# lzzcd001/MeshDiffusion

Measured on AMD Instinct MI355X. Metric: denoise steps/sec on 64^3x4 DMTet grids (sample-steps/s = n_gpus*batch*steps/wall), higher is better.
Workload: dtype f16f6 in the Winograd convs behind a GroupNorm (fp16 hi*hi MFMA + MX block-scaled e2m3 cross terms in a K-concatenated scaled MFMA at twice the e4m3 rate; operands and weights equalised per input channel by a power of two: md_wino_equaliser, after the load-time calibration from the measured operand

## Files before the change

include/meshdiffusion_hip.h:

```cpp
#ifndef MESHDIFFUSION_HIP_H
#define MESHDIFFUSION_HIP_H

#include <stdint.h>

#ifdef __cplusplus
extern "C" {
#endif

#define MD_OK 0
#define MD_ERR_BAD_ARG (-1)
#define MD_ERR_UNSUPPORTED (-2)
#define MD_ERR_NO_DEVICE (-3)

#define MD_ABI_VERSION 16

enum {
  MD_CFG_C3_128 = 0,
  MD_CFG_C3_128_K16 = 1,
  MD_CFG_C3_32 = 2,
  MD_CFG_C3_LOW = 3,
  MD_CFG_C3_S2 = 4,
  MD_CFG_G1_128 = 5,
  MD_CFG_G1_128_LOW = 6,
  MD_CFG_G1_64_LOW = 7,
// ... 129 lines not shown
int md_wino_prep_f6(const float* x1, const float* x2, int32_t c1, int32_t c2, const float* ac, int32_t silu, int32_t ups,
                    const float* eq, void* t_out, int32_t batch, int32_t D, int32_t H, int32_t W, void* stream);
int md_wino_pack_weights_f6(const float* w, const float* eq, void* wpk, int32_t cout, int32_t cin, int64_t s_row, int64_t s_k, void* stream);
int md_conv3_wino_f6(const void* t_in, const void* wpk, float* out, const float* bias, int64_t bias_bstride,
                     const float* residual, int64_t res_bstride, double* stats, int32_t batch, int32_t cin, int32_t cout,
                     int32_t D, int32_t H, int32_t W, void* stream);

int md_wino_prep_f6_nin(const float* x1, const float* x2, int32_t c1, int32_t c2, const float* ac, int32_t silu, const float* eq,
                        void* t_out, const void* wpk, const float* bias, float* res, int32_t batch, int32_t D, int32_t H, int32_t W,
                        int32_t n_cu, void* stream);

#define MD_WINO_FMT_BF16X3 0
#define MD_WINO_FMT_F16F8 1
#define MD_WINO_FMT_F16F6 2
int md_wino_prep_upsdh(int32_t fmt, const float* x1, const float* x2, int32_t c1, int32_t c2, const float* ac, int32_t silu,
                       const float* eq, void* t_out, int32_t batch, int32_t D, int32_t H, int32_t W, void* stream);
int md_conv3_wino_upsdh(int32_t fmt, const void* t_in, const void* wpk, float* out, const float* bias, int64_t bias_bstride,
                        const float* residual, int64_t res_bstride, double* stats, int32_t batch, int32_t cin, int32_t cout,
                        int32_t D, int32_t H, int32_t W, void* stream);

int md_conv3_wino_upsfold(int32_t fmt, const void* t_in, int32_t t_full, const void* wpk, float* out, const float* bias,
                          int64_t bias_bstride, const float* residual, int64_t res_bstride, double* stats, int32_t batch,
                          int32_t cin, int32_t cout, int32_t D, int32_t H, int32_t W, void* stream);

int md_conv3_stem(const void* x16, const void* wpk, float* out, const float* bias, const float* residual, double* stats,
                  int32_t batch, int32_t cout, int32_t D, int32_t H, int32_t W, void* stream);

int md_conv3_head(const float* x, const float* ac, const void* wpk, float* y, int32_t batch, int32_t cin, int32_t rows_alloc,
                  int32_t D, int32_t H, int32_t W, void* stream);

int md_conv3_stem_dgrad(const float* g0, const void* wpk, float* y, int32_t batch, int32_t cout, int32_t rows_alloc,
                        int32_t D, int32_t H, int32_t W, void* stream);

enum { MD_PACK_WPK = 0, MD_PACK_WINO = 1, MD_PACK_WINO_F6 = 2 };
typedef struct MdPackJob {
  const float* w;
  void* out;
  int64_t s_row, s_k, s_tap, n_items, block0;
  int32_t rows, kdim, taps, nt, kc, prec, flip, kind;
} MdPackJob;
int md_pack_batch(const MdPackJob* jobs_dev, int32_t n_jobs, int64_t total_blocks, int32_t tiled, void* stream);

int md_conv3_s2(const float* x, const void* wpk, float* out, const float* bias, int64_t bias_bstride, double* stats,
                int32_t batch, int32_t cin, int32_t rows, int32_t rows_alloc, int32_t D, int32_t H, int32_t W, void* stream);

int md_wino_prep_v2(const float* x1, const float* x2, int32_t c1, int32_t c2, const float* ac, int32_t silu, int32_t ups,
// ... 281 lines not shown
```

meshdiffusion_amd/csrc/conv3_wino.hip:

```cpp
#include <type_traits>
#include "md_common.h"
#include "md_pack.h"

namespace {
constexpr int WN_THREADS = 256;
constexpr int WN_TZ = 4, WN_TY = 8, WN_TX = 8;
constexpr int WN_TPOS = 6 * 10 * 4;
constexpr int WN_HBUF = 4 * WN_TPOS * 16;
constexpr int WN_NDMA = WN_HBUF / 1024;
constexpr int WN_RED = 4 * 32 * 2;
constexpr int WN_WAVE_LDS = 2 * WN_HBUF;
constexpr int WN_LDS_BYTES = 4 * WN_WAVE_LDS + 4 * WN_NDMA * 64 * 4;

__device__ const uint4 wn_zero16 = {0u, 0u, 0u, 0u};

typedef uint32_t wn_u32x4 __attribute__((ext_vector_type(4)));
__device__ __forceinline__ uint4 wn_gload16(const void* p) {
  return __builtin_bit_cast(uint4, *(__attribute__((address_space(1))) const wn_u32x4*)(uintptr_t)p);
}
}

__global__ __launch_bounds__(256) void md_wino_prep_kernel(const float* __restrict__ x1, const float* __restrict__ x2,
                                                           int c1, int c2, const float* __restrict__ ac, int silu, int ups,
                                                           uint4* __restrict__ T, int batch, int D, int H, int W,
// ... 114 lines not shown
  const float wscale = md_wino_f8_wscale(__uint_as_float(hdr[0]));
  if (id == 0) {
    hdr[1] = (uint32_t)ilogbf(wscale);
    hdr[2] = __float_as_uint(1.0f / wscale);
    hdr[3] = 6u;
  }
  if (id >= n) return;
  wpk[id] = md_pack_wino_f6_item(w, cout, cin, s_row, s_k, wscale, id, eq);
}

struct WnArgs {
  const uint4* T;
  const uint4* wpk;
  float* out;
  const float* bias;
  const float* residual;
  double* stats;
  const float* hdr;
  int64_t bias_bstride, res_bstride;
  int batch, cin, cout, D, H, W;
  float out_scale;
  const uint32_t* amax;
  int ups_dh;
};

typedef int wn_i32x8 __attribute__((ext_vector_type(8)));
typedef int wn_i32x4 __attribute__((ext_vector_type(4)));

template <int ABL, bool F8 = false, bool F6 = false, bool RES = false>
__global__ __launch_bounds__(WN_THREADS) void md_conv3_wino_kernel(const WnArgs A) {
  __shared__ __attribute__((aligned(16))) unsigned char wn_smem[WN_LDS_BYTES];
  const int tid = threadIdx.x, lane = tid & 63;
  const int wid = __builtin_amdgcn_readfirstlane(tid >> 6);
  const int j = lane & 31, h = lane >> 5;
  uint64_t stamp[12];
  auto mark = [&](int k) { if constexpr (ABL & 128) stamp[k] = __builtin_amdgcn_s_memtime(); };
  if constexpr (ABL & 128) stamp[10] = __builtin_amdgcn_s_memrealtime();
  mark(0);

#ifndef W8_STAGGER
#define W8_STAGGER 0
#endif
  if constexpr (W8_STAGGER > 0) {
    const unsigned lin = blockIdx.x + gridDim.x * blockIdx.y;
    if (lin < 256u) {
      const unsigned ph = (lin * 0x9E3779B1u) >> 24;
      const uint64_t t_end = __builtin_amdgcn_s_memtime() + ((uint64_t)ph * (uint64_t)W8_STAGGER >> 8);
      while (__builtin_amdgcn_s_memtime() < t_end) __builtin_amdgcn_s_sleep(16);
    }
  }
  const int D = A.D, H = A.H, W = A.W, Wp = W >> 1;
  const int64_t P = (int64_t)D * H * W, Ph = P >> (1 + 2 * A.ups_dh);
  const int ush = A.ups_dh, Hrows = H >> ush;
  const int ntx = W / WN_TX, nty = H / WN_TY, ntz = D / WN_TZ;
  const int tiles = ntx * nty * ntz;
  int bid = blockIdx.x;
  if ((gridDim.x & 7) == 0) bid = (blockIdx.x & 7) * (gridDim.x >> 3) + (blockIdx.x >> 3);
  const int b = bid / tiles, t = bid % tiles;
  const int x0 = (t % ntx) * WN_TX, y0 = ((t / ntx) % nty) * WN_TY, z0 = (t / (ntx * nty)) * WN_TZ;
  const int rtb = blockIdx.y;
  const int CG = A.cin >> 3, nchunk = A.cin >> 4;
  const int nsteps = nchunk * 9;

  unsigned char* my_smem = wn_smem + wid * WN_WAVE_LDS;

  auto halo_off = [&](int k) -> int {
    const int e = k * 64 + lane;
    const int hp = e / WN_TPOS, tp = e % WN_TPOS;
    const int dz = tp / 40, hy = (tp >> 2) % 10, pr = tp & 3;
    const int z = z0 + dz - 1, y = y0 + hy - 1;
    const bool live = (z >= 0) & (z < D) & (y >= 0) & (y < H);
    const int row = (z >> ush) * Hrows + (y >> ush);
    if constexpr (F8) {
      const int Phi = (int)Ph;
      const int off = (hp >> 1) * 8 * Phi + (hp & 1) * Phi + row * Wp + (x0 >> 1) + pr;
      return live ? off : -1;
    }
    return live ? (int)((int64_t)(hp >> 1) * 8 * Ph + (int64_t)(hp & 1) * Ph + (int64_t)row * Wp + (x0 >> 1) + pr) : -1;
  };
  const uint4* tbase = A.T + ((int64_t)b * CG * 8 + wid * 2) * Ph;
  const uint4* zsrc = &wn_zero16;
  auto halo_load = [&](int chunk, int k) -> uint4 {
    const int dk = halo_off(k);
    const uint4* src = dk >= 0 ? tbase + (int64_t)chunk * 16 * Ph + dk : zsrc;
    if constexpr (ABL & 32)
      src = A.T + (((blockIdx.x & 255) * 4 + wid) * 2 + (chunk & 1)) * 960 + k * 64 + lane;
    if constexpr (ABL & 64)
      src = A.T + ((((((int64_t)bid * 4 + wid) * nchunk + chunk) * 960) & (((int64_t)1 << 26) - 1)) + k * 64 + lane);
    if constexpr (ABL & 1) return make_uint4(0, 0, 0, 0);
    return wn_gload16(src);
  };
  auto halo_store = [&](int buf, int k, const uint4& v) {
    if constexpr (!(ABL & 1)) *(uint4*)(my_smem + buf * WN_HBUF + k * 1024 + lane * 16) = v;
  };
  const uint4* wbase = A.wpk + (((int64_t)rtb * nsteps) * 4 + wid) * 512 + lane;
  auto load_A = [&](int s, bf16x8 (&dst)[8]) {
    const uint4* wp = wbase + (int64_t)s * 2048;
#pragma unroll
    for (int i = 0; i < 8; ++i) dst[i] = __builtin_bit_cast(bf16x8, wp[i * 64]);
  };
  const unsigned char* vB = my_smem + h * 2 * WN_TPOS * 16 + j * 16;
  auto read_B = [&](int tap, int buf, bf16x8 (&dst)[8], bool force) {
    const int kd = tap / 3, kh = tap % 3;
    const unsigned char* p = vB + buf * WN_HBUF + (kd * 40 + kh * 4) * 16;
#pragma unroll
    for (int ct = 0; ct < 4; ++ct)
      if (force || !(ABL & 8)) {
        dst[ct * 2] = *(const bf16x8*)(p + ct * 40 * 16);
        dst[ct * 2 + 1] = *(const bf16x8*)(p + WN_TPOS * 16 + ct * 40 * 16);
      }
  };

  f32x16 acc[4][4];
  auto zero_acc = [&]() {
#pragma unroll
    for (int rt = 0; rt < 4; ++rt)
#pragma unroll
      for (int ct = 0; ct < 4; ++ct) {
#pragma unroll
        for (int r = 0; r < 16; ++r) acc[rt][ct][r] = 0.f;
        asm volatile("" : "+a"(acc[rt][ct]));
      }
  };
#ifndef W8_PRO_FENCE
#define W8_PRO_FENCE 1
#endif
  if constexpr (!W8_PRO_FENCE) zero_acc();
  float descale = 1.f;
  if constexpr (F8) {
    static_assert(ABL == 0 || ABL == 128, "timing ablations exist for the bf16x3 loop only");
#ifndef W8_HG
#define W8_HG 3
#endif
    auto slot3_of_store = [](int u) constexpr -> int { return (u == 0 || u == 3 || u == 6) ? 0 : ((u == 2 || u == 5 || u == 8) ? 1 : 2); };
    auto slot3_of_request = [](int u) constexpr -> int { return (u == 0 || u == 3 || u == 6) ? 0 : ((u == 2 || u == 5 || u == 8) ? 1 : 2); };
    const int npairs = nsteps >> 1;
    const uint4* wbase8 = A.wpk + (((int64_t)rtb * npairs) * 4 + wid) * 1024 + lane;
    uint4 A8h[2][4][2], B8h[2][2], hs8[W8_HG == 3 ? 3 : 2][4];
    wn_i32x8 A8f[2][4], B8f[2];
    uint32_t* otab = (uint32_t*)(wn_smem + 4 * WN_WAVE_LDS) + wid * (WN_NDMA * 64) + lane;
    static_assert(4 * WN_WAVE_LDS + 4 * WN_NDMA * 64 * 4 <= WN_LDS_BYTES, "offset tables fit behind the halo buffers");
    uint32_t live_mask = 0;
    constexpr int D1 = 64, D2 = (40 - 8) * 16, D3 = WN_HBUF - (2 * 40 + 2 * 4) * 16;
    const unsigned char* vBh = my_smem + h * 2 * WN_TPOS * 16 + j * 16;
    const unsigned char* vB8a = my_smem + WN_TPOS * 16 + j * 16 + h * D1;
    const unsigned char* vB8b = my_smem + WN_TPOS * 16 + j * 16 + h * D2;
    const unsigned char* vB8c = my_smem + WN_TPOS * 16 + j * 16 + h * D3;
    auto step_off = [](int s) constexpr -> int { return (s / 9) * WN_HBUF + (((s % 9) / 3) * 40 + ((s % 9) % 3) * 4) * 16; };
    auto cat8 = [](const uint4& x, const uint4& y) -> wn_i32x8 {
      const wn_i32x4 a = __builtin_bit_cast(wn_i32x4, x), b = __builtin_bit_cast(wn_i32x4, y);
      return __builtin_shufflevector(a, b, 0, 1, 2, 3, 4, 5, 6, 7);
    };
    auto halo_store8 = [&](int buf, int k, uint4 v) {
      const bool lv = (live_mask >> k) & 1u;
      v.x = lv ? v.x : 0u; v.y = lv ? v.y : 0u; v.z = lv ? v.z : 0u; v.w = lv ? v.w : 0u;
      *(uint4*)(my_smem + buf * WN_HBUF + k * 1024 + lane * 16) = v;
    };
    auto read_B8 = [&](auto uc, auto ctc, uint4 (&dh)[2], wn_i32x8& df) {
      constexpr int u = decltype(uc)::value, ct = decltype(ctc)::value;
      constexpr int o0 = step_off(2 * u) + ct * 40 * 16, o1 = step_off(2 * u + 1) + ct * 40 * 16, dk = o1 - o0;
// ... 254 lines not shown
        __builtin_amdgcn_sched_group_barrier(0x008, 2, 0);
        __builtin_amdgcn_sched_group_barrier(0x200, 1, 0);
        __builtin_amdgcn_sched_barrier(0);
      }
    }
  #undef WN_MFMA
  }

  mark(2);
  if constexpr (ABL & 16) {
    float keep = 0.f;
#pragma unroll
    for (int rt = 0; rt < 4; ++rt)
#pragma unroll
      for (int ct = 0; ct < 4; ++ct) keep += acc[rt][ct][0];
    if (keep == 123.456f) A.out[tid] = keep;
    return;
  }
  constexpr int XF_ITEMS = 1024, XREG_FLOATS = (4 * XF_ITEMS + 16) * 4;
  static_assert(2 * XREG_FLOATS * 4 + 2 * WN_RED * 4 <= WN_LDS_BYTES, "two exchange regions + the statistics area fit");
  float* xreg = (float*)wn_smem;
  float* red = xreg + 2 * XREG_FLOATS;
  const int rows_total = A.cout;
  float* outp = A.out + (int64_t)b * rows_total * P;
  const float* resp = A.residual ? A.residual + (int64_t)b * A.res_bstride : nullptr;
  const float* biasp = A.bias ? A.bias + (int64_t)b * A.bias_bstride : nullptr;
  const bool want_stats = (ABL & 128) ? false : A.stats != nullptr;
  const int half = lane & 1, xq = (lane >> 1) & 7, cgp = lane >> 4;
  const int cq = 2 * cgp + half, prr = xq >> 1;
  const bool odd = xq & 1;
  const float sgn = odd ? -1.f : 1.f;
  const int64_t gp0 = ((int64_t)(z0 + wid) * H + y0) * W + x0 + xq;
  auto flush_stats = [&](int r) {
    if (tid < 64) {
      const int ch = tid >> 1, which = tid & 1;
      const float* rb = red + (r & 1) * WN_RED;
      float sum = 0.f;
#pragma unroll
      for (int k = 0; k < 4; ++k) sum += rb[(k * 32 + ch) * 2 + which];
      const int row = rtb * 128 + r * 32 + ch;
      atomicAdd(A.stats + ((int64_t)b * rows_total + row) * 2 + which, (double)sum);
    }
  };
  const bool has_bias = biasp != nullptr;
  f32x4 pbias[4], pres[RES ? 2 : 1][8];
  auto prefetch_res = [&](int r) {
    if constexpr (RES) {
// ... 183 lines not shown
extern "C" int md_wino_pack_weights_f8(const float* w, const float* eq, void* wpk, int32_t cout, int32_t cin, int64_t s_row, int64_t s_k, void* stream) {
  return md_wino_pack_weights_f8_launch(false, w, eq, wpk, cout, cin, s_row, s_k, stream);
}

extern "C" int md_wino_pack_weights_f6(const float* w, const float* eq, void* wpk, int32_t cout, int32_t cin, int64_t s_row, int64_t s_k, void* stream) {
  return md_wino_pack_weights_f8_launch(true, w, eq, wpk, cout, cin, s_row, s_k, stream);
}

static int md_conv3_wino_f8_launch(bool f6, const void* t_in, const void* wpk, float* out, const float* bias, int64_t bias_bstride,
                                   const float* residual, int64_t res_bstride, double* stats, int32_t batch, int32_t cin,
                                   int32_t cout, int32_t D, int32_t H, int32_t W, void* stream, float out_scale = 1.0f,
                                   const uint32_t* amax = nullptr, bool upsdh = false) {
  if (!t_in || !wpk || !out || batch <= 0) return MD_ERR_BAD_ARG;
  if (cin <= 0 || cout <= 0 || (cin % 32) || (cout % 128)) return MD_ERR_UNSUPPORTED;
  if (D <= 0 || H <= 0 || W <= 0 || (D % WN_TZ) || (H % WN_TY) || (W % WN_TX)) return MD_ERR_UNSUPPORTED;
  if ((int64_t)D * H * W * 8 >= (int64_t)1 << 31) return MD_ERR_UNSUPPORTED;
  WnArgs a;
  a.T = (const uint4*)t_in; a.wpk = (const uint4*)wpk; a.out = out; a.bias = bias; a.residual = residual; a.stats = stats;
  a.hdr = (const float*)((const unsigned char*)wpk + (int64_t)cout * cin * 36 * 4);
  a.out_scale = out_scale; a.amax = amax;
  a.bias_bstride = bias_bstride; a.res_bstride = res_bstride;
  a.batch = batch; a.cin = cin; a.cout = cout; a.D = D; a.H = H; a.W = W;
  a.ups_dh = upsdh ? 1 : 0;
  const int tiles = (D / WN_TZ) * (H / WN_TY) * (W / WN_TX);
  const dim3 grid((unsigned)(tiles * batch), (unsigned)(cout / 128));
  MD_HIP_CLEAR_ERROR();
#ifdef W8_STAMPS
  constexpr int ABL_ = 128;
#else
  constexpr int ABL_ = 0;
#endif
#define WN_LAUNCH8(F6_, RES_) hipLaunchKernelGGL((md_conv3_wino_kernel<ABL_, true, F6_, RES_>), grid, dim3(WN_THREADS), 0, (hipStream_t)stream, a)
  if (f6) { if (residual) WN_LAUNCH8(true, true); else WN_LAUNCH8(true, false); }
  else { if (residual) WN_LAUNCH8(false, true); else WN_LAUNCH8(false, false); }
#undef WN_LAUNCH8
  MD_HIP_CHECK_LAUNCH();
  return MD_OK;
}

extern "C" int md_conv3_wino_f8(const void* t_in, const void* wpk, float* out, const float* bias, int64_t bias_bstride,
                                const float* residual, int64_t res_bstride, double* stats, int32_t batch, int32_t cin,
                                int32_t cout, int32_t D, int32_t H, int32_t W, void* stream) {
  return md_conv3_wino_f8_launch(false, t_in, wpk, out, bias, bias_bstride, residual, res_bstride, stats, batch, cin, cout, D, H, W, stream);
}

extern "C" int md_conv3_wino_f6(const void* t_in, const void* wpk, float* out, const float* bias, int64_t bias_bstride,
// ... 4 lines not shown

extern "C" int md_conv3_wino_f6_scaled(const void* t_in, const void* wpk, float* out, const float* bias, int64_t bias_bstride,
                                       const float* residual, int64_t res_bstride, double* stats, int32_t batch, int32_t cin,
                                       int32_t cout, int32_t D, int32_t H, int32_t W, float out_scale, const uint32_t* amax_bits, void* stream) {
  if (!(out_scale > 0.f)) return MD_ERR_BAD_ARG;
  return md_conv3_wino_f8_launch(true, t_in, wpk, out, bias, bias_bstride, residual, res_bstride, stats, batch, cin, cout, D, H, W, stream, out_scale,
                                 amax_bits);
}

static int md_conv3_wino_launch(const void* t_in, const void* wpk, float* out, const float* bias, int64_t bias_bstride,
                                const float* residual, int64_t res_bstride, double* stats, int32_t batch, int32_t cin,
                                int32_t cout, int32_t D, int32_t H, int32_t W, int32_t variant, void* stream, bool upsdh) {
  if (!t_in || !wpk || !out || batch <= 0) return MD_ERR_BAD_ARG;
  if (cin <= 0 || cout <= 0 || (cin % 32) || (cout % 128)) return MD_ERR_UNSUPPORTED;
  if (D <= 0 || H <= 0 || W <= 0 || (D % WN_TZ) || (H % WN_TY) || (W % WN_TX)) return MD_ERR_UNSUPPORTED;
  if ((int64_t)D * H * W * 8 >= (int64_t)1 << 31) return MD_ERR_UNSUPPORTED;
  WnArgs a;
  a.T = (const uint4*)t_in; a.wpk = (const uint4*)wpk; a.out = out; a.bias = bias; a.residual = residual; a.stats = stats;
  a.hdr = nullptr;
  a.out_scale = 1.0f; a.amax = nullptr;
  a.bias_bstride = bias_bstride; a.res_bstride = res_bstride;
  a.batch = batch; a.cin = cin; a.cout = cout; a.D = D; a.H = H; a.W = W;
  a.ups_dh = upsdh ? 1 : 0;
  const int tiles = (D / WN_TZ) * (H / WN_TY) * (W / WN_TX);
  MD_HIP_CLEAR_ERROR();
  const dim3 grid((unsigned)(tiles * batch), (unsigned)(cout / 128));
#define WN_LAUNCH(A_) hipLaunchKernelGGL((md_conv3_wino_kernel<A_, false, false, true>), grid, dim3(WN_THREADS), 0, (hipStream_t)stream, a)
  if (variant != 0 && residual == nullptr) return MD_ERR_UNSUPPORTED;
  if (upsdh && variant != 0) return MD_ERR_BAD_ARG;
  switch (variant) {
    case 0:
      if (residual) WN_LAUNCH(0);
      else hipLaunchKernelGGL((md_conv3_wino_kernel<0, false, false, false>), grid, dim3(WN_THREADS), 0, (hipStream_t)stream, a);
      break;
#ifdef MD_BUILD_ABLATIONS
    case 1: WN_LAUNCH(1); break;
    case 2: WN_LAUNCH(2); break;
    case 4: WN_LAUNCH(4); break;
    case 6: WN_LAUNCH(6); break;
    case 22: WN_LAUNCH(22); break;
    case 9: WN_LAUNCH(9); break;
    case 16: WN_LAUNCH(16); break;
    case 25: WN_LAUNCH(25); break;
    case 32: WN_LAUNCH(32); break;
    case 64: WN_LAUNCH(64); break;
    case 128: WN_LAUNCH(128); break;
#endif
    default: return MD_ERR_UNSUPPORTED;
  }
#undef WN_LAUNCH
  MD_HIP_CHECK_LAUNCH();
  return MD_OK;
}

extern "C" int md_conv3_wino(const void* t_in, const void* wpk, float* out, const float* bias, int64_t bias_bstride,
                             const float* residual, int64_t res_bstride, double* stats, int32_t batch, int32_t cin,
                             int32_t cout, int32_t D, int32_t H, int32_t W, int32_t variant, void* stream) {
  return md_conv3_wino_launch(t_in, wpk, out, bias, bias_bstride, residual, res_bstride, stats, batch, cin, cout, D, H, W, variant, stream, false);
}

extern "C" int md_conv3_wino_upsdh(int32_t fmt, const void* t_in, const void* wpk, float* out, const float* bias, int64_t bias_bstride,
                                   const float* residual, int64_t res_bstride, double* stats, int32_t batch, int32_t cin,
                                   int32_t cout, int32_t D, int32_t H, int32_t W, void* stream) {
  if (fmt == MD_WINO_FMT_BF16X3)
    return md_conv3_wino_launch(t_in, wpk, out, bias, bias_bstride, residual, res_bstride, stats, batch, cin, cout, D, H, W, 0, stream, true);
  if (fmt != MD_WINO_FMT_F16F8 && fmt != MD_WINO_FMT_F16F6) return MD_ERR_BAD_ARG;
  return md_conv3_wino_f8_launch(fmt == MD_WINO_FMT_F16F6, t_in, wpk, out, bias, bias_bstride, residual, res_bstride, stats, batch, cin, cout, D, H,
                                 W, stream, 1.0f, nullptr, true);
}
```

meshdiffusion_amd/csrc/gemm_conv.hip:

```cpp
#include "md_common.h"
#include "md_pack.h"

template <int NT_, int KC_, int TZ_, int TY_, int TX_, int TAPS_, int STRIDE_, int WR_, int WC_,
          int SW_ = 0, int PIPE_ = 0, int ABL_ = 0, int BF_ = 0>
struct GCfg {
  static constexpr int BF = BF_;
  static constexpr int ABL = ABL_;
  static constexpr int NT = NT_, KC = KC_, TZ = TZ_, TY = TY_, TX = TX_, TAPS = TAPS_,
                       STRIDE = STRIDE_, WR = WR_, WC = WC_, SW = SW_, PIPE = PIPE_;
  static constexpr int MT = TZ * TY * TX;
  static constexpr int NW = WR * WC;
  static constexpr int NTHREADS = NW * 64;
  static constexpr int RM = NT / (32 * WR);
  static constexpr int CM = MT / (32 * WC);
  static constexpr int KSZ = (TAPS == 125 || TAPS == 25) ? 5 : (TAPS == 27 || TAPS == 9) ? 3 : 1;
  static constexpr int KSX = (TAPS == 25 || TAPS == 9) ? 1 : KSZ;
  static constexpr int ZH = (TAPS > 1) ? (TZ - 1) * STRIDE + KSZ : 1;
  static constexpr int YH = (TAPS > 1) ? (TY - 1) * STRIDE + KSZ : 1;
  static constexpr int XH = (TAPS > 1) ? (TX - 1) * STRIDE + KSX : MT;
  static constexpr int XHP = XH;
  static constexpr int HS = (SW == 1) ? ((ZH + 1) / 2) * YH * 24 : ZH * YH * XHP;
  static constexpr int HPOS = ZH * YH * XH;
  static __device__ __forceinline__ int slot_of(int hz, int hy, int hx) {
    if constexpr (SW == 1) return (hz >> 1) * (YH * 24) + hy * 24 + (hz & 1) * 12 + hx;
// ... 541 lines not shown
  }
  __syncthreads();
  if (threadIdx.x < 16) {
    const float t = (red[0][threadIdx.x] + red[1][threadIdx.x]) + (red[2][threadIdx.x] + red[3][threadIdx.x]);
    A.stats[((int64_t)b * A.rows_alloc + cg * 8) * 2 + threadIdx.x] += (double)t;
  }
}

int md_launch_splitk_reduce(const MdGemmConvArgs& a, hipStream_t stream) {
  const int64_t P = (int64_t)a.D * a.H * a.W;
  if (a.stats != nullptr) {
    MD_HIP_CLEAR_ERROR();
    hipLaunchKernelGGL(md_splitk_reduce_stats_kernel, dim3((unsigned)(a.batch * (a.rows_alloc / 8))), dim3(256), 0, stream, a, P);
    MD_HIP_CHECK_LAUNCH();
    return MD_OK;
  }
  const int64_t n4 = (int64_t)a.batch * (a.rows_alloc / 8) * P * 2;
  int blocks = (int)((n4 + 255) / 256);
  if (blocks > 2048) blocks = 2048;
  MD_HIP_CLEAR_ERROR();
  hipLaunchKernelGGL(md_splitk_reduce_kernel, dim3((unsigned)blocks), dim3(256), 0, stream, a, P);
  MD_HIP_CHECK_LAUNCH();
  return MD_OK;
}

extern "C" int64_t md_gemm_conv_partial_bytes(const MdGemmConvArgs* a) {
  if (a == nullptr) return MD_ERR_BAD_ARG;
  if (a->ksplit <= 1) return 0;
  return (int64_t)a->ksplit * a->batch * (a->rows_alloc / 8) * ((int64_t)a->D * a->H * a->W) * 8 * 4;
}

template <class C>
static int launch_cfg(const MdGemmConvArgs& a, hipStream_t stream) {
  if (a.kdim % C::KC != 0 || a.kdim <= 0) return MD_ERR_BAD_ARG;
  if (a.rows <= 0 || a.rows_alloc % 8 != 0 || a.batch <= 0) return MD_ERR_BAD_ARG;
  int tiles;
  if (C::TAPS > 1) {
    if (a.D % C::TZ || a.H % C::TY || a.W % C::TX) return MD_ERR_BAD_ARG;
    if (a.ups && ((a.D | a.H | a.W) & 1)) return MD_ERR_BAD_ARG;
    if (a.ups && C::STRIDE != 1) return MD_ERR_BAD_ARG;
    tiles = (a.D / C::TZ) * (a.H / C::TY) * (a.W / C::TX);
  } else {
    if (a.D != 1 || a.H != 1 || a.W % C::MT || a.ups) return MD_ERR_BAD_ARG;
    tiles = a.W / C::MT;
  }
  if (a.a_src == MD_A_S16B && a.a_rows <= 0) return MD_ERR_BAD_ARG;
// ... 137 lines not shown
```

meshdiffusion_amd/hip_ops.py:

```python
import ctypes as C
import math
import os

import torch

from . import _lib
from ._lib import (A_PACKED, A_S16B, PREC_BF16X3, PREC_FP16X2, CFG_C3_128, CFG_C3_128_V2, CFG_C3_128_SW, CFG_C3_128_PIPE, CFG_C3_128_FAST, CFG_C5_128_K16, CFG_C5_32_K16, CFG_C3_128_W4, CFG_C3X_32, CFG_C5X_32_K16, CFG_C3X_128_K16, CFG_C5X_128, CFG_G1_128_N128, CFG_C3_128_K16, CFG_C3_32, CFG_C3_LOW, CFG_C3_S2,
                   CFG_G1_128, CFG_G1_128_LOW, CFG_G1_64_LOW, CFG_NT_KC, OUT_F32B, OUT_NCDHW, OUT_S16B,
                   MdGemmConvArgs, check)


CFG_ABL1, CFG_ABL2, CFG_ABL3, CFG_ABL4, CFG_ABL5 = 101, 102, 103, 104, 105
CFG_F1, CFG_F3, CFG_F4, CFG_F6, CFG_F7, CFG_F8 = 111, 113, 114, 116, 117, 118
CFG_FAST_EC = 122
_MODES = ("bf16x3", "fp16x2", "f16f8", "f16f6")
DEFAULT_PRECISION = os.environ.get("MD_PRECISION", "bf16x3")
FORCE_PRECISION = os.environ.get("MD_FORCE_PRECISION")
WINO_EQ = os.environ.get("MD_WINO_EQ", "1") == "1"


def _decode(mode):
    if mode not in _MODES:
        raise ValueError(f"unknown precision mode {mode!r}")
    return ("bf16x3", mode[3:]) if mode in ("f16f8", "f16f6") else (mode, False)
# ... 465 lines not shown
CALIBRATE = None


def wino_operand_ms(parts, ac, silu, B, P):
    lib = _lib.load()
    assert 1 <= len(parts) <= 2
    cin = sum(c for _, c in parts)
    x2, c2 = (parts[1][0], parts[1][1]) if len(parts) == 2 else (None, 0)
    ms = torch.zeros(cin, dtype=torch.float32, device=parts[0][0].device)
    check(lib.md_wino_operand_ms(_ptr(parts[0][0]), _ptr(x2), parts[0][1], c2, _ptr(ac), 1 if silu else 0, B, P, _ptr(ms), _stream()),
          "md_wino_operand_ms")
    return ms


WINO_MIN_WGS = 128
WINO_MIN_WGS_TRAIN = 256


def wino_ok(rows, kdim, S, B):
    return (WINO and PRECISION == "bf16x3" and rows % 128 == 0 and kdim % 32 == 0 and S % 8 == 0
            and B * (S ** 3 // 256) * (rows // 128) >= (max(WINO_MIN_WGS, WINO_MIN_WGS_TRAIN) if TRAINING_SCOPE else WINO_MIN_WGS))


def wgrad_nin_ok(co, ci, P):
    return co % 128 == 0 and ci % 128 == 0 and P % 16 == 0


def wgrad_nin(dy_s16, x_s16, B, co, ci, P, dw, ksplit=None):
    lib = _lib.load()
    units = (co // 128) * (ci // 128)
    if ksplit is None:
        ksplit = max(1, min(256 // units, B * P // 16 // 8))
    nbytes = lib.md_wgrad_nin_workspace_bytes(co, ci, ksplit)
    if nbytes <= 0:
        raise _lib.MeshDiffusionHipError("md_wgrad_nin_workspace_bytes: unsupported shape")
    ws = torch.empty(nbytes // 4, dtype=torch.float32, device=dy_s16.device)
    ev = _prof_begin()
    check(lib.md_wgrad_nin(_ptr(dy_s16), _ptr(x_s16), _ptr(dw), _ptr(ws), nbytes, B, co, ci, P, ksplit, 1, co, _stream()),
          "md_wgrad_nin")
    _prof_end(ev, "wgrad_nin", 2.0 * B * co * ci * P, 4.0 * B * (co + ci) * P, f"{ci}->{co}@{P}")


_WINO_SCRATCH = {}


def _wino_scratch(n_bf16, device, slot="t"):
# ... 146 lines not shown


def conv3_wino_upsfold(wf, t, B, S, *, bias=None, bias_bstride=0, stats=None, out=None, dims=None):
    lib = _lib.load()
    D, H, W = dims if dims is not None else (S, S, S)
    P = D * H * W
    assert isinstance(wf, WinoWeightF8) and wf.fmt == "f6" and wf.rows % 4 == 0
    rows = wf.rows // 4
    t_fmt = getattr(t, "_md_fmt", None)
    if t_fmt is not None:
        if t_fmt != "f6" or not getattr(t, "_md_ups", False) or getattr(t, "_md_eq", 0) != (wf.eq.data_ptr() if wf.eq is not None else 0):
            raise _lib.MeshDiffusionHipError(f"conv3_wino_upsfold: operand (format {t_fmt!r}) does not belong to these weights")
    if out is None:
        out = f32b_empty(B, rows, P, t.device)
    ev = _prof_begin()
    check(lib.md_conv3_wino_upsfold(_lib.WINO_FMT["f6"], _ptr(t), 0 if getattr(t, "_md_compact", False) else 1, _ptr(wf.data), _ptr(out),
                                    _ptr(bias), bias_bstride, None, 0, _ptr(stats), B, wf.kdim, rows, D, H, W, _stream()),
          "md_conv3_wino_upsfold")
    _prof_end(ev, "wino", 2.0 * B * rows * wf.kdim * 27 * P, 4.0 * (2 * B * wf.kdim * P // 4 + wf.rows * wf.kdim * 36 + B * rows * P),
              f"{wf.kdim}->{rows}@{D}x{H}x{W}" + ("/stats" if stats is not None else "") + "/fold/f6")
    return out


CFG_S2_PACK = CFG_C3_128_K16
S2_MIN_WGS = 100


def conv3_s2_ok(rows, kdim, S_out, B=None):
    ok = PRECISION == "bf16x3" and kdim % 32 == 0 and rows % 8 == 0 and S_out % 8 == 0
    return ok and (B is None or B * (S_out ** 3 // 256) * ((rows + 127) // 128) >= S2_MIN_WGS)


def conv3_s2(pw, x, B, S_out, *, bias=None, bias_bstride=0, stats=None, out=None, dims=None):
    lib = _lib.load()
    D, H, W = dims if dims is not None else (S_out, S_out, S_out)
    P = D * H * W
    rows_alloc = ((pw.rows + 7) // 8) * 8
    if out is None:
        out = f32b_empty(B, rows_alloc, P, x.device)
    ev = _prof_begin()
    check(lib.md_conv3_s2(_ptr(x), _ptr(pw.data), _ptr(out), _ptr(bias), bias_bstride, _ptr(stats), B, pw.kdim, pw.rows,
                          rows_alloc, D, H, W, _stream()), "md_conv3_s2")
    _prof_end(ev, "s2", 2.0 * B * pw.rows * pw.kdim * 27 * P, 4.0 * (B * pw.kdim * 8 * P + pw.rows * pw.kdim * 27 + B * pw.rows * P),
              f"{pw.kdim}->{pw.rows}@{D}x{H}x{W}" + ("/stats" if stats is not None else ""))
    return out

# ... 539 lines not shown
```

meshdiffusion_amd/lib/diffusion/models/layers.py:

```python
import math
from typing import NamedTuple

import numpy as np
import torch
import torch.nn as nn

from .... import hip_ops as ops


def variance_scaling(scale, mode, distribution, in_axis=1, out_axis=0, dtype=torch.float32, device="cpu"):
    def init(shape, dtype=dtype, device=device):
        receptive = np.prod(shape) / shape[in_axis] / shape[out_axis]
        fan_in, fan_out = shape[in_axis] * receptive, shape[out_axis] * receptive
        denom = {"fan_in": fan_in, "fan_out": fan_out, "fan_avg": (fan_in + fan_out) / 2}[mode]
        var = scale / denom
        if distribution == "normal":
            return torch.randn(*shape, dtype=dtype, device=device) * np.sqrt(var)
        if distribution == "uniform":
            return (torch.rand(*shape, dtype=dtype, device=device) * 2.0 - 1.0) * np.sqrt(3 * var)
        raise ValueError("invalid distribution for variance scaling initializer")

    return init


# ... 108 lines not shown


def fused_operand_ok(pw, ups=0):
    cfgs = (ops.CFG_C3_128_FAST,) if ups else (ops.CFG_C3_128_FAST, ops.CFG_C3_LOW)
    return ops.FUSE_GN_APPLY and pw.cfg in cfgs and pw.prec == ops.PREC_BF16X3


class Conv3Plan(NamedTuple):
    path: str
    fmt: object
    compact: bool
    shortcut_in_pass: bool
    keep: bool
    stats: bool
    ksplit: int
    fused_loader: bool
    ups_fold: bool = False


def plan_conv3(pw, operand, B, S_out, *, ups, out_mode, rows_alloc, want_stats, wino):
    P = S_out ** 3
    plain = out_mode == ops.OUT_F32B and rows_alloc == pw.rows
    sums = bool(want_stats and ops.FUSE_GN_STATS and plain)
    if (operand is not None and wino is not None and plain and pw.prec == ops.PREC_BF16X3
            and ops.wino_ok(pw.rows, pw.kdim, S_out, B)):
        infer = not (operand.wino_only or operand.drop or operand.keep)
        fmt = infer and ops.wino_f8_ok(
            S_out, parts=operand.parts, normalised=operand.ac is not None
            or (ops.WINO_EQ and hasattr(wino, "measured") and wino.measured() is not None))
        owner = getattr(wino, "owner", None)
        if fmt and owner is not None and wino.site in getattr(owner, "md_bf16x3_sites", ()):
            fmt = False
        compact = infer and ops.prep_compact_ok(ups, S_out, S_out, S_out)
        shortcut = bool(operand.nin is not None and fmt == "f6" and not compact and not ups
                        and ops.block_pass_ok(operand.parts, operand.nin[0].rows, B, S_out, S_out, S_out))
        fold = bool(infer and hasattr(wino, "fold") and ops.ups_fold_ok(ups, fmt, pw.rows, B, S_out, S_out, S_out))
        return Conv3Plan("wino", fmt, compact, shortcut, operand.keep, sums, 1, False, fold)
    ksplit = ops.ksplit_for(pw.cfg, B, pw.rows, pw.kdim, S_out) if out_mode == ops.OUT_F32B else 1
    sums = sums and ((pw.cfg == ops.CFG_C3_128_FAST and ksplit == 1) or (ksplit > 1 and P <= 512 and B * rows_alloc >= 2048))
    return Conv3Plan("direct", False, False, False, False, sums, ksplit, operand is not None and not operand.wino_only)


def run_conv3(pw, act_s16, B, S_out, *, bias=None, bias_bstride=0, residual=None, res_bstride=None, ups=0,
              out=None, out_mode=ops.OUT_F32B, rows_alloc=None, want_stats=False, b_f32=None, wino=None):
    P = S_out ** 3
    b_f32 = ops.F32Operand.of(b_f32)
    dev = act_s16.device if act_s16 is not None else b_f32.parts[0][0].device
    rows_alloc = rows_alloc if rows_alloc is not None else ((pw.rows + 7) // 8) * 8
    if out is None:
        out = ops.f32b_empty(B, rows_alloc, P, dev)
    if residual is not None and res_bstride is None:
        res_bstride = rows_alloc * P
    if b_f32 is not None:
        b_f32.t_kept = b_f32.shortcut = None
    plan = plan_conv3(pw, b_f32, B, S_out, ups=ups, out_mode=out_mode, rows_alloc=rows_alloc, want_stats=want_stats, wino=wino)
    stats = ops.stats_zeros(B, rows_alloc, dev) if plan.stats else None
    if plan.path == "wino":
        _conv3_wino(plan, pw, b_f32, wino, B, S_out, ups, out, stats, bias=bias, bias_bstride=bias_bstride, residual=residual,
                    res_bstride=res_bstride or 0)
    else:
# ... 6 lines not shown
    elif hasattr(out, "_md_sums"):
        del out._md_sums
    return out


def _conv3_wino(plan, pw, op, wino, B, S_out, ups, out, stats, **epilogue):
    owner = getattr(wino, "owner", None)
    if ops.CALIBRATE is not None and owner is not None and not op.wino_only:
        ms = ops.wino_operand_ms(op.parts, op.ac, op.silu, B, op.parts[0][0].shape[2])
        rec = ops.CALIBRATE.setdefault((id(owner), wino.site), [owner, wino.site, torch.zeros_like(ms), 0])
        rec[2] += ms
        rec[3] += 1
    eq = wino.eq() if plan.fmt and hasattr(wino, "eq") else None
    if plan.shortcut_in_pass:
        t, op.shortcut = ops.wino_prep_nin(op.parts, op.ac, op.silu, B, S_out, eq, op.nin[0], op.nin[1])
    else:
        t = ops.wino_prep(op.parts, op.ac, op.silu, ups, B, S_out, drop=op.drop, keep=plan.keep, f8=plan.fmt, eq=eq, compact=plan.compact)
    if plan.keep:
        op.t_kept = t
    if plan.ups_fold:
        assert epilogue.get("residual") is None, "md_conv3_wino_upsfold has no residual operand"
        ops.conv3_wino_upsfold(wino.fold(), t, B, S_out, stats=stats, out=out, bias=epilogue.get("bias"),
                               bias_bstride=epilogue.get("bias_bstride", 0))
    else:
        ops.conv3_wino(wino(plan.fmt) if plan.fmt else wino(), t, B, S_out, stats=stats, out=out, **epilogue)
    if plan.fmt and ops.AUDIT is not None:
        t3 = ops.wino_prep(op.parts, op.ac, op.silu, ups, B, S_out, compact=plan.compact)
        ref = ops.conv3_wino(wino(), t3, B, S_out, **epilogue)
        ops.AUDIT.append(dict(owner=owner, site=getattr(wino, "site", None), fmt=plan.fmt, cin=pw.kdim, cout=pw.rows,
                              S=S_out, rel_l2=float((torch.linalg.vector_norm(out - ref, dtype=torch.float64)
                                                     / torch.linalg.vector_norm(ref, dtype=torch.float64).clamp_min(1e-300)).item())))


def run_gemm(pw, act_s16, B, P, *, bias=None, bias_bstride=0, residual=None, out=None, out_mode=ops.OUT_F32B,
             alpha=1.0, b_bstride=None, b_f32=None):
    rows_alloc = ((pw.rows + 7) // 8) * 8
    b_f32 = ops.F32Operand.of(b_f32)
    dev = act_s16.device if act_s16 is not None else b_f32.parts[0][0].device
    if out is None:
        out = (ops.f32b_empty if out_mode == ops.OUT_F32B else ops.s16b_empty)(B, rows_alloc, P, dev)
    return ops.gemm_conv(cfg=pw.cfg, a=pw.data, b=act_s16, out=out, batch=B, rows=pw.rows,
                         rows_alloc=rows_alloc, kdim=pw.kdim, dims=(1, 1, P), bias=bias,
                         bias_bstride=bias_bstride, residual=residual,
                         res_bstride=rows_alloc * P if residual is not None else 0, alpha=alpha,
                         out_mode=out_mode, b_bstride=b_bstride, b_f32=b_f32)

# ... 311 lines not shown
```

Before: 118.3.

## Add split-K Winograd conv path for small 8^3 layers with too few workgroups

Adds a split-K variant of the Winograd conv kernel. The input-channel reduction is divided into ksplit slices, each writing partial sums to a workspace, and the existing split-K reduce kernel then applies bias, residual and stats. The planner picks this path for inference at S=8 when the workgroup count falls below the normal Winograd threshold, aiming to fill more CUs on small layers. The cost is an extra workspace allocation per call, an additional reduce launch and extra memory traffic for the partials.

After: 120.0 (median of 6 runs). 1.4% higher.

```diff
diff --git a/include/meshdiffusion_hip.h b/include/meshdiffusion_hip.h
--- a/include/meshdiffusion_hip.h
+++ b/include/meshdiffusion_hip.h
@@ -175,6 +175,11 @@
 int md_conv3_wino_upsfold(int32_t fmt, const void* t_in, int32_t t_full, const void* wpk, float* out, const float* bias,
                           int64_t bias_bstride, const float* residual, int64_t res_bstride, double* stats, int32_t batch,
                           int32_t cin, int32_t cout, int32_t D, int32_t H, int32_t W, void* stream);
+
+int64_t md_conv3_wino_splitk_workspace_bytes(int32_t batch, int32_t cout, int32_t D, int32_t H, int32_t W, int32_t ksplit);
+int md_conv3_wino_splitk(int32_t fmt, const void* t_in, const void* wpk, void* workspace, int64_t workspace_bytes, float* out,
+                         const float* bias, int64_t bias_bstride, const float* residual, int64_t res_bstride, double* stats,
+                         int32_t batch, int32_t cin, int32_t cout, int32_t D, int32_t H, int32_t W, int32_t ksplit, void* stream);
 
 int md_conv3_stem(const void* x16, const void* wpk, float* out, const float* bias, const float* residual, double* stats,
                   int32_t batch, int32_t cout, int32_t D, int32_t H, int32_t W, void* stream);
diff --git a/meshdiffusion_amd/csrc/conv3_wino.hip b/meshdiffusion_amd/csrc/conv3_wino.hip
--- a/meshdiffusion_amd/csrc/conv3_wino.hip
+++ b/meshdiffusion_amd/csrc/conv3_wino.hip
@@ -1,5 +1,6 @@
 #include <type_traits>
 #include "md_common.h"
+#include "md_args.h"
 #include "md_pack.h"
 
 namespace {
@@ -160,6 +161,7 @@
   float out_scale;
   const uint32_t* amax;
   int ups_dh;
+  int ks, nsteps_full;
 };
 
 typedef int wn_i32x8 __attribute__((ext_vector_type(8)));
@@ -194,7 +196,8 @@
   const int tiles = ntx * nty * ntz;
   int bid = blockIdx.x;
   if ((gridDim.x & 7) == 0) bid = (blockIdx.x & 7) * (gridDim.x >> 3) + (blockIdx.x >> 3);
-  const int b = bid / tiles, t = bid % tiles;
+  const int bp = bid / tiles, t = bid % tiles;
+  const int sl = RES ? 0 : bp % A.ks, b = RES ? bp : bp / A.ks;
   const int x0 = (t % ntx) * WN_TX, y0 = ((t / ntx) % nty) * WN_TY, z0 = (t / (ntx * nty)) * WN_TZ;
   const int rtb = blockIdx.y;
   const int CG = A.cin >> 3, nchunk = A.cin >> 4;
@@ -216,7 +219,7 @@
     }
     return live ? (int)((int64_t)(hp >> 1) * 8 * Ph + (int64_t)(hp & 1) * Ph + (int64_t)row * Wp + (x0 >> 1) + pr) : -1;
   };
-  const uint4* tbase = A.T + ((int64_t)b * CG * 8 + wid * 2) * Ph;
+  const uint4* tbase = A.T + ((int64_t)bp * CG * 8 + wid * 2) * Ph;
   const uint4* zsrc = &wn_zero16;
   auto halo_load = [&](int chunk, int k) -> uint4 {
     const int dk = halo_off(k);
@@ -231,7 +234,7 @@
   auto halo_store = [&](int buf, int k, const uint4& v) {
     if constexpr (!(ABL & 1)) *(uint4*)(my_smem + buf * WN_HBUF + k * 1024 + lane * 16) = v;
   };
-  const uint4* wbase = A.wpk + (((int64_t)rtb * nsteps) * 4 + wid) * 512 + lane;
+  const uint4* wbase = A.wpk + (((int64_t)rtb * A.nsteps_full + sl * nsteps) * 4 + wid) * 512 + lane;
   auto load_A = [&](int s, bf16x8 (&dst)[8]) {
     const uint4* wp = wbase + (int64_t)s * 2048;
 #pragma unroll
@@ -273,7 +276,7 @@
     auto slot3_of_store = [](int u) constexpr -> int { return (u == 0 || u == 3 || u == 6) ? 0 : ((u == 2 || u == 5 || u == 8) ? 1 : 2); };
     auto slot3_of_request = [](int u) constexpr -> int { return (u == 0 || u == 3 || u == 6) ? 0 : ((u == 2 || u == 5 || u == 8) ? 1 : 2); };
     const int npairs = nsteps >> 1;
-    const uint4* wbase8 = A.wpk + (((int64_t)rtb * npairs) * 4 + wid) * 1024 + lane;
+    const uint4* wbase8 = A.wpk + (((int64_t)rtb * (A.nsteps_full >> 1) + sl * npairs) * 4 + wid) * 1024 + lane;
     uint4 A8h[2][4][2], B8h[2][2], hs8[W8_HG == 3 ? 3 : 2][4];
     wn_i32x8 A8f[2][4], B8f[2];
     uint32_t* otab = (uint32_t*)(wn_smem + 4 * WN_WAVE_LDS) + wid * (WN_NDMA * 64) + lane;
@@ -574,7 +577,7 @@
   float* xreg = (float*)wn_smem;
   float* red = xreg + 2 * XREG_FLOATS;
   const int rows_total = A.cout;
-  float* outp = A.out + (int64_t)b * rows_total * P;
+  float* outp = A.out + ((int64_t)sl * A.batch + b) * rows_total * P;
   const float* resp = A.residual ? A.residual + (int64_t)b * A.res_bstride : nullptr;
   const float* biasp = A.bias ? A.bias + (int64_t)b * A.bias_bstride : nullptr;
   const bool want_stats = (ABL & 128) ? false : A.stats != nullptr;
@@ -804,6 +807,7 @@
   a.bias_bstride = bias_bstride; a.res_bstride = res_bstride;
   a.batch = batch; a.cin = cin; a.cout = cout; a.D = D; a.H = H; a.W = W;
   a.ups_dh = upsdh ? 1 : 0;
+  a.ks = 1; a.nsteps_full = (cin / 16) * 9;
   const int tiles = (D / WN_TZ) * (H / WN_TY) * (W / WN_TX);
   const dim3 grid((unsigned)(tiles * batch), (unsigned)(cout / 128));
   MD_HIP_CLEAR_ERROR();
@@ -854,6 +858,7 @@
   a.bias_bstride = bias_bstride; a.res_bstride = res_bstride;
   a.batch = batch; a.cin = cin; a.cout = cout; a.D = D; a.H = H; a.W = W;
   a.ups_dh = upsdh ? 1 : 0;
+  a.ks = 1; a.nsteps_full = (cin / 16) * 9;
   const int tiles = (D / WN_TZ) * (H / WN_TY) * (W / WN_TX);
   MD_HIP_CLEAR_ERROR();
   const dim3 grid((unsigned)(tiles * batch), (unsigned)(cout / 128));
@@ -900,3 +905,48 @@
   return md_conv3_wino_f8_launch(fmt == MD_WINO_FMT_F16F6, t_in, wpk, out, bias, bias_bstride, residual, res_bstride, stats, batch, cin, cout, D, H,
                                  W, stream, 1.0f, nullptr, true);
 }
+
+int md_splitk_finish(const float* partial, float* out, const float* bias, int64_t bias_bstride, const float* residual, int64_t res_bstride,
+                     double* stats, int batch, int rows, int D, int H, int W, int ksplit, hipStream_t stream);
+
+extern "C" int64_t md_conv3_wino_splitk_workspace_bytes(int32_t batch, int32_t cout, int32_t D, int32_t H, int32_t W, int32_t ksplit) {
+  if (batch <= 0 || cout <= 0 || (cout & 7) || D <= 0 || H <= 0 || W <= 0 || ksplit < 2) return MD_ERR_BAD_ARG;
+  return (int64_t)ksplit * batch * cout * ((int64_t)D * H * W) * 4;
+}
+
+extern "C" int md_conv3_wino_splitk(int32_t fmt, const void* t_in, const void* wpk, void* workspace, int64_t workspace_bytes, float* out,
+                                    const float* bias, int64_t bias_bstride, const float* residual, int64_t res_bstride, double* stats,
+                                    int32_t batch, int32_t cin, int32_t cout, int32_t D, int32_t H, int32_t W, int32_t ksplit, void* stream) {
+  if (fmt != MD_WINO_FMT_BF16X3 && fmt != MD_WINO_FMT_F16F8 && fmt != MD_WINO_FMT_F16F6) return MD_ERR_BAD_ARG;
+  if (md_any_bad<16>(t_in, wpk, workspace, out) || md_any_misaligned<16>(residual) || md_any_misaligned<4>(bias) ||
+      md_any_misaligned<8>(stats))
+    return MD_ERR_BAD_ARG;
+  if (batch <= 0 || ksplit < 2 || bias_bstride < 0 || res_bstride < 0 || (res_bstride & 3)) return MD_ERR_BAD_ARG;
+  if (cin <= 0 || cout <= 0 || (cout % 128) || (cin % (32 * (int64_t)ksplit))) return MD_ERR_UNSUPPORTED;
+  if (D <= 0 || H <= 0 || W <= 0 || (D % WN_TZ) || (H % WN_TY) || (W % WN_TX)) return MD_ERR_UNSUPPORTED;
+  const int64_t P = (int64_t)D * H * W;
+  if (P * 8 >= (int64_t)1 << 31) return MD_ERR_UNSUPPORTED;
+  const int64_t tiles = (D / WN_TZ) * (int64_t)(H / WN_TY) * (W / WN_TX);
+  if (!md_fits_i32(tiles * batch * ksplit, (int64_t)batch * ksplit) || cout / 128 > 65535 || batch * (cout / 8) > 0x7fffffffLL)
+    return MD_ERR_UNSUPPORTED;
+  if (workspace_bytes < (int64_t)ksplit * batch * cout * P * 4) return MD_ERR_BAD_ARG;
+  WnArgs a;
+  a.T = (const uint4*)t_in; a.wpk = (const uint4*)wpk; a.out = (float*)workspace; a.bias = nullptr; a.residual = nullptr; a.stats = nullptr;
+  a.hdr = fmt == MD_WINO_FMT_BF16X3 ? nullptr : (const float*)((const unsigned char*)wpk + (int64_t)cout * cin * 36 * 4);
+  a.out_scale = 1.0f; a.amax = nullptr;
+  a.bias_bstride = 0; a.res_bstride = 0;
+  a.batch = batch; a.cin = cin / ksplit; a.cout = cout; a.D = D; a.H = H; a.W = W;
+  a.ups_dh = 0;
+  a.ks = ksplit; a.nsteps_full = (cin / 16) * 9;
+  const dim3 grid((unsigned)(tiles * batch * ksplit), (unsigned)(cout / 128));
+  MD_HIP_CLEAR_ERROR();
+  if (fmt == MD_WINO_FMT_BF16X3)
+    hipLaunchKernelGGL((md_conv3_wino_kernel<0, false, false, false>), grid, dim3(WN_THREADS), 0, (hipStream_t)stream, a);
+  else if (fmt == MD_WINO_FMT_F16F8)
+    hipLaunchKernelGGL((md_conv3_wino_kernel<0, true, false, false>), grid, dim3(WN_THREADS), 0, (hipStream_t)stream, a);
+  else
+    hipLaunchKernelGGL((md_conv3_wino_kernel<0, true, true, false>), grid, dim3(WN_THREADS), 0, (hipStream_t)stream, a);
+  MD_HIP_CHECK_LAUNCH();
+  return md_splitk_finish((const float*)workspace, out, bias, bias_bstride, residual, res_bstride, stats, batch, cout, D, H, W, ksplit,
+                          (hipStream_t)stream);
+}
diff --git a/meshdiffusion_amd/csrc/gemm_conv.hip b/meshdiffusion_amd/csrc/gemm_conv.hip
--- a/meshdiffusion_amd/csrc/gemm_conv.hip
+++ b/meshdiffusion_amd/csrc/gemm_conv.hip
@@ -587,6 +587,17 @@
   hipLaunchKernelGGL(md_splitk_reduce_kernel, dim3((unsigned)blocks), dim3(256), 0, stream, a, P);
   MD_HIP_CHECK_LAUNCH();
   return MD_OK;
+}
+
+int md_splitk_finish(const float* partial, float* out, const float* bias, int64_t bias_bstride, const float* residual, int64_t res_bstride,
+                     double* stats, int batch, int rows, int D, int H, int W, int ksplit, hipStream_t stream) {
+  if (!partial || !out || batch <= 0 || rows <= 0 || (rows & 7) || ksplit < 1 || D <= 0 || H <= 0 || W <= 0) return MD_ERR_BAD_ARG;
+  MdGemmConvArgs a = {};
+  a.partial = const_cast<float*>(partial); a.out = out; a.bias = bias; a.residual = residual; a.stats = stats;
+  a.bias_bstride = bias_bstride; a.res_bstride = res_bstride;
+  a.alpha = 1.0f; a.batch = batch; a.rows = rows; a.rows_alloc = rows; a.D = D; a.H = H; a.W = W; a.ksplit = ksplit;
+  a.out_mode = MD_OUT_F32B;
+  return md_launch_splitk_reduce(a, stream);
 }
 
 extern "C" int64_t md_gemm_conv_partial_bytes(const MdGemmConvArgs* a) {
diff --git a/meshdiffusion_amd/hip_ops.py b/meshdiffusion_amd/hip_ops.py
--- a/meshdiffusion_amd/hip_ops.py
+++ b/meshdiffusion_amd/hip_ops.py
@@ -511,6 +511,25 @@
             and B * (S ** 3 // 256) * (rows // 128) >= (max(WINO_MIN_WGS, WINO_MIN_WGS_TRAIN) if TRAINING_SCOPE else WINO_MIN_WGS))
 
 
+WINO_SPLITK = os.environ.get("MD_WINO_SPLITK", "1") == "1"
+WINO_SPLITK_MIN_WGS = 64
+WINO_SPLITK_MAX_WGS = 256
+WINO_SPLITK_MIN_K = 256
+
+
+def wino_splitk_for(rows, kdim, S, B, ups=0):
+    if not (WINO_SPLITK and WINO and PRECISION == "bf16x3" and not TRAINING_SCOPE and not ups and S == 8
+            and rows % 128 == 0 and kdim % 32 == 0 and kdim >= WINO_SPLITK_MIN_K):
+        return 0
+    n = B * (S ** 3 // 256) * (rows // 128)
+    if not (WINO_SPLITK_MIN_WGS <= n < WINO_MIN_WGS):
+        return 0
+    for ks in (8, 4, 2):
+        if kdim % (32 * ks) == 0 and n * ks <= WINO_SPLITK_MAX_WGS:
+            return ks
+    return 0
+
+
 def wgrad_nin_ok(co, ci, P):
     return co % 128 == 0 and ci % 128 == 0 and P % 16 == 0
 
@@ -703,6 +722,35 @@
     return out
 
 
+def conv3_wino_splitk(ww, t, B, S, ksplit, *, bias=None, bias_bstride=0, residual=None, res_bstride=0, stats=None, out=None, dims=None):
+    lib = _lib.load()
+    D, H, W = dims if dims is not None else (S, S, S)
+    P = D * H * W
+    f8 = isinstance(ww, WinoWeightF8)
+    assert f8 or isinstance(ww, WinoWeight), "the weights of conv3_wino (no scaled data-gradient form)"
+    t_fmt = getattr(t, "_md_fmt", None)
+    if t_fmt is not None:
+        want = ww.fmt if f8 else False
+        if (t_fmt != want or getattr(t, "_md_compact", False)
+                or getattr(t, "_md_eq", 0) != ((ww.eq.data_ptr() if ww.eq is not None else 0) if f8 else 0)):
+            raise _lib.MeshDiffusionHipError(f"conv3_wino_splitk: operand format {t_fmt!r} / equaliser does not belong to these weights ({want!r})")
+    if out is None:
+        out = f32b_empty(B, ww.rows, P, t.device)
+    nbytes = lib.md_conv3_wino_splitk_workspace_bytes(B, ww.rows, D, H, W, ksplit)
+    if nbytes <= 0:
+        raise _lib.MeshDiffusionHipError("md_conv3_wino_splitk_workspace_bytes: unsupported shape")
+    ws = torch.empty(nbytes // 4, dtype=torch.float32, device=t.device)
+    ev = _prof_begin()
+    check(lib.md_conv3_wino_splitk(_lib.WINO_FMT[ww.fmt if f8 else False], _ptr(t), _ptr(ww.data), _ptr(ws), nbytes, _ptr(out), _ptr(bias),
+                                   bias_bstride, _ptr(residual), res_bstride, _ptr(stats), B, ww.kdim, ww.rows, D, H, W, ksplit, _stream()),
+          "md_conv3_wino_splitk")
+    _prof_end(ev, "wino_splitk", 2.0 * B * ww.rows * ww.kdim * 27 * P,
+              4.0 * (2 * B * ww.kdim * P + ww.rows * ww.kdim * 36 + B * ww.rows * P * (2 * ksplit + (2 if residual is not None else 1))),
+              f"{ww.kdim}->{ww.rows}@{D}x{H}x{W}/ks{ksplit}" + ("/res" if residual is not None else "") + ("/stats" if stats is not None else "")
+              + (("/" + ww.fmt) if f8 else ""))
+    return out
+
+
 CFG_S2_PACK = CFG_C3_128_K16
 S2_MIN_WGS = 100
 
diff --git a/meshdiffusion_amd/lib/diffusion/models/layers.py b/meshdiffusion_amd/lib/diffusion/models/layers.py
--- a/meshdiffusion_amd/lib/diffusion/models/layers.py
+++ b/meshdiffusion_amd/lib/diffusion/models/layers.py
@@ -154,9 +154,11 @@
     P = S_out ** 3
     plain = out_mode == ops.OUT_F32B and rows_alloc == pw.rows
     sums = bool(want_stats and ops.FUSE_GN_STATS and plain)
-    if (operand is not None and wino is not None and plain and pw.prec == ops.PREC_BF16X3
-            and ops.wino_ok(pw.rows, pw.kdim, S_out, B)):
-        infer = not (operand.wino_only or operand.drop or operand.keep)
+    infer = operand is not None and not (operand.wino_only or operand.drop or operand.keep)
+    wino_ks = 0
+    if operand is not None and wino is not None and plain and pw.prec == ops.PREC_BF16X3:
+        wino_ks = 1 if ops.wino_ok(pw.rows, pw.kdim, S_out, B) else (ops.wino_splitk_for(pw.rows, pw.kdim, S_out, B, ups) if infer else 0)
+    if wino_ks:
         fmt = infer and ops.wino_f8_ok(
             S_out, parts=operand.parts, normalised=operand.ac is not None
             or (ops.WINO_EQ and hasattr(wino, "measured") and wino.measured() is not None))
@@ -167,7 +169,7 @@
         shortcut = bool(operand.nin is not None and fmt == "f6" and not compact and not ups
                         and ops.block_pass_ok(operand.parts, operand.nin[0].rows, B, S_out, S_out, S_out))
         fold = bool(infer and hasattr(wino, "fold") and ops.ups_fold_ok(ups, fmt, pw.rows, B, S_out, S_out, S_out))
-        return Conv3Plan("wino", fmt, compact, shortcut, operand.keep, sums, 1, False, fold)
+        return Conv3Plan("wino", fmt, compact, shortcut, operand.keep, sums, wino_ks, False, fold)
     ksplit = ops.ksplit_for(pw.cfg, B, pw.rows, pw.kdim, S_out) if out_mode == ops.OUT_F32B else 1
     sums = sums and ((pw.cfg == ops.CFG_C3_128_FAST and ksplit == 1) or (ksplit > 1 and P <= 512 and B * rows_alloc >= 2048))
     return Conv3Plan("direct", False, False, False, False, sums, ksplit, operand is not None and not operand.wino_only)
@@ -220,6 +222,8 @@
         assert epilogue.get("residual") is None, "md_conv3_wino_upsfold has no residual operand"
         ops.conv3_wino_upsfold(wino.fold(), t, B, S_out, stats=stats, out=out, bias=epilogue.get("bias"),
                                bias_bstride=epilogue.get("bias_bstride", 0))
+    elif plan.ksplit > 1:
+        ops.conv3_wino_splitk(wino(plan.fmt) if plan.fmt else wino(), t, B, S_out, plan.ksplit, stats=stats, out=out, **epilogue)
     else:
         ops.conv3_wino(wino(plan.fmt) if plan.fmt else wino(), t, B, S_out, stats=stats, out=out, **epilogue)
     if plan.fmt and ops.AUDIT is not None:
```
